# TravisWheelerLab/BATH

Hardware: AMD Instinct MI355X
Metric: DP Gcells/s + residues/s through bathsearch pipeline at 1/2/4/8 MI355X (higher is better)
Workload: dtype u8/i16 integer scores (SSV: exact binary16), f32 Forward

## Files before the change

### bath_amd/csrc/bath_common.hpp

```cpp
#pragma once
#include <set>
#include <atomic>
#include <hip/hip_runtime.h>

#include <cstdint>
#include <chrono>
#include <cstdio>
#include <cstdlib>
#include <cstring>
#include <condition_variable>
#include <functional>
#include <mutex>
#include <shared_mutex>
#include <string>
#include <thread>
#include <vector>

#include "bath_hip.h"

namespace bath {

inline hipError_t allow_max_lds(const void *fn) {
  static std::mutex mu;
  static std::set<std::pair<int, const void *>> done;
  int dev = 0;
  (void)hipGetDevice(&dev);
  std::lock_guard<std::mutex> g(mu);
  if (done.count({dev, fn})) return hipSuccess;
  hipFuncAttributes at{};
  size_t fixed = 0;
  if (hipFuncGetAttributes(&at, fn) == hipSuccess) fixed = at.sharedSizeBytes; else (void)hipGetLastError();
  const hipError_t e = hipFuncSetAttribute(fn, hipFuncAttributeMaxDynamicSharedMemorySize, (int)(160 * 1024 - (int)std::min<size_t>(fixed, 96 * 1024)));
  if (e == hipSuccess) done.insert({dev, fn});
  return e;
}

constexpr int kKp = BATH_KP_AMINO;
constexpr int kRowReset = 29;
constexpr int kSsvRows = 30;
constexpr int kStop = 27;
constexpr int kXaa = 26;
constexpr int kOrfBins = 2048;
constexpr int kOrfCursorStride = 32;
constexpr int kOrfMiscInts = (1 + kOrfCursorStride) * kOrfBins + 64;

#define BATH_HIP_TRY(ctx, call)                                                            \
  do {                                                                                     \
    hipError_t e_ = (call);                                                                \
    if (e_ != hipSuccess) {                                                                \
      (ctx)->set_error(std::string(#call) + ": " + hipGetErrorString(e_));                 \
      return BATH_EFAIL;                                                                   \
    }                                                                                      \
  } while (0)

struct DevBuf {
  void *p = nullptr;
  size_t cap = 0;
  hipError_t reserve(size_t bytes) {
    if (bytes <= cap) return hipSuccess;
    if (p) (void)hipFree(p);
    p = nullptr; cap = 0;
    size_t want = bytes + bytes / 4 + 256;
// ... 246 lines not shown
  uint64_t uid = 0;
  int M = 0, max_length = 0, L0 = 0;
  float nj = 1.f;
  float evparam[BATH_NEVPARAM];
  float compo[BATH_K_AMINO];
  std::vector<uint8_t> rb;
  std::vector<int16_t> rw;
  std::vector<int16_t> tw;
  std::vector<float> rf, tf;
  uint8_t tbm_b = 0, tec_b = 0, base_b = 0, bias_b = 0;
  float scale_b = 0;
  int16_t xw_E[2] = {0, 0};
  float scale_w = 0;
  int16_t base_w = 0, ddbound_w = 0;
  float xf_E[2] = {0, 0};
  std::string consensus;
  std::vector<uint8_t> cons_digital;
  uint8_t *d_cons = nullptr;
  std::vector<float> prefix_lengths, suffix_lengths;
  int NR = 0, G = 1;
  int ssv_row_bytes = 0;
  int16_t *d_ssv = nullptr;
  int16_t *d_msv = nullptr;
  uint8_t *d_rb = nullptr;
  int rb_stride = 0;
  int16_t *d_rw = nullptr;
  int16_t *d_tw = nullptr;
  float *d_rf = nullptr, *d_tf = nullptr;
  float *d_rfb = nullptr, *d_tfb = nullptr;
  float *d_msc = nullptr, *d_tsc = nullptr;
  float *d_bias_eo = nullptr;
  int vit_NR = 0, vit_rw_pitch = 0;
  int16_t *d_vit_rw = nullptr; uint32_t *d_vit_tw2 = nullptr; int16_t *d_vit_rank = nullptr;
  mutable LenTables lt;
  mutable std::mutex grow_mu;
  mutable std::vector<void *> retired;
  mutable int16_t *d_emit = nullptr;
  mutable double emit_F1 = -1.0;
  mutable int emit_maxlen = -1;
  int ensure_len_tables(int maxL) const;
};

namespace bath {
int build_len_tables(const bath_hip_oprofile *om, int maxL);
void bias_filter_eo(const float *compo, float eo[kKp][2]);
double gumbel_surv(double x, double mu, double lambda);
// ... 15 lines not shown
```

### bath_amd/csrc/bath_filters.hip

```cpp
#include <cmath>
#include <cstring>
#include <algorithm>
#include <numeric>

#include "bath_common.hpp"
#include "bath_kernels.hpp"
#include "bath_launch.hpp"

using namespace bath;

namespace bath {


template <int NR, int G>
__global__ __launch_bounds__(256, NR <= 76 ? 4 : 1) void ssv_lane_kernel(SeqView sq, const int32_t *__restrict__ order,
                                                       const int16_t *__restrict__ cost_tab, int row_bytes,
                                                       int16_t *__restrict__ out_v) {
  extern __shared__ __attribute__((aligned(16))) char lds[];
  {
    const int n32 = kSsvRows * row_bytes / 4;
    const uint32_t *src = reinterpret_cast<const uint32_t *>(cost_tab);
    uint32_t *dst = reinterpret_cast<uint32_t *>(lds);
    for (int i = threadIdx.x; i < n32; i += blockDim.x) dst[i] = src[i];
  }
  __syncthreads();
  const int64_t gt = (int64_t)blockIdx.x * blockDim.x + threadIdx.x;
  const int lane_ = threadIdx.x & 63;
  const int64_t t = (gt >> 6) * (64 / G) + SsvGroups<G>::slot(lane_);
  const int grank = SsvGroups<G>::rank(lane_);
  const bool live = t < sq.n;
  const int64_t sid = live ? (order ? (int64_t)order[t] : t) : 0;
  const int L = live ? sq.len[sid] : 0;
  const uint8_t *s = sq.data + sq.off[sid];
  const int Lw = wave_max_i32(L);
  const char *tile = lds + grank * (4 * NR);
  const unsigned tile_addr = (unsigned)(size_t)(__attribute__((address_space(3))) const char *)tile;

  s16x2 reg[NR];
  const s16x2 fl = {0, 0};
#pragma unroll
  for (int r = 0; r < NR; r++) reg[r] = fl;
  s16x2 xE = fl, xE2 = fl;

  uint32_t wnext = (0 < L) ? *reinterpret_cast<const uint32_t *>(s) : 0x1d1d1d1du;
  for (int i0 = 0; i0 < Lw; i0 += 4) {
    const uint32_t w = wnext;
    wnext = (i0 + 4 < L) ? *reinterpret_cast<const uint32_t *>(s + i0 + 4) : 0x1d1d1d1du;
#pragma unroll 1
    for (int j = 0; j < 4; j++) {
      int x = (w >> (8 * j)) & 0xff;
      x = (i0 + j < L) ? min(x, kKp - 1) : kRowReset;
      const unsigned carry = ssv_carry<NR, G>(reg, grank);
      ssv_row_pipe<NR, 3>(reg, xE, xE2, tile_addr + (unsigned)(x * row_bytes), carry);
    }
  }
  xE = ssv_max3(xE, xE2, xE2);
  const int v = ssv_group_max<G>(xE);
  if (live && grank == 0) out_v[sid] = (int16_t)min(v, 32767);
}

__global__ void ssv_classify_kernel(int64_t n, const int32_t *__restrict__ len, const int16_t *__restrict__ v,
                                    const uint8_t *__restrict__ tjb_tab, MsvConsts c, float *__restrict__ sc,
                                    int32_t *__restrict__ status) {
  const int64_t t = (int64_t)blockIdx.x * blockDim.x + threadIdx.x;
  if (t >= n) return;
  float s = 0.f;
  const int st = ssv_classify(v[t], tjb_tab[len[t]], c, &s);
  sc[t] = s;
  status[t] = st;
}

template <int C>
__global__ __launch_bounds__(256) void msv_wave_kernel(SeqView sq, int M, const uint8_t *__restrict__ rb, int rb_stride,
                                                       const uint8_t *__restrict__ tjb_tab, MsvConsts c,
                                                       const int32_t *__restrict__ todo, int64_t ntodo, const int *__restrict__ ntodo_dev,
                                                       float *__restrict__ sc, int32_t *__restrict__ status) {
// ... 576 lines not shown
  c.base_w = om->base_w; c.xwE_loop = om->xw_E[0]; c.xwE_move = om->xw_E[1]; c.scale_w = om->scale_w;
  c.scale_b = om->scale_b; c.base_b = om->base_b; c.tec_b = om->tec_b; c.bias_b = om->bias_b;
  c.Q8 = std::max(2, ((om->M - 1) / 8) + 1);
  return c;
}

static int length_order(bath_hip_ctx *ctx, const bath_hip_seqs *sq, DevBuf &buf) {
  std::vector<int32_t> order((size_t)sq->n);
  std::iota(order.begin(), order.end(), 0);
  std::stable_sort(order.begin(), order.end(), [&](int32_t a, int32_t b) { return sq->h_len[a] > sq->h_len[b]; });
  BATH_HIP_TRY(ctx, buf.reserve(order.size() * sizeof(int32_t) + 16));
  BATH_HIP_TRY(ctx, hipMemcpyAsync(buf.p, order.data(), order.size() * sizeof(int32_t), hipMemcpyHostToDevice, ctx->stream));
  return BATH_OK;
}

int launch_ssv_lane(bath_hip_ctx *ctx, const bath_hip_oprofile *om, SeqView v, const int32_t *d_order, int16_t *d_v) {
  if (v.n == 0) return BATH_OK;
  const int G = om->G;
  const size_t shmem = (size_t)kSsvRows * om->ssv_row_bytes;
  const int threads = 256;
  const int blocks = (int)((v.n * G + threads - 1) / threads);
  const int rb = om->ssv_row_bytes;
  bool launched = false;
#define BATH_SSV_CASE(N, GG)                                                                                             \
  if (!launched && om->NR == N && G == GG) {                                                                             \
    if (shmem > 64 * 1024) (void)bath::allow_max_lds((const void *)ssv_lane_kernel<N, GG>); \
    hipLaunchKernelGGL((ssv_lane_kernel<N, GG>), dim3(blocks), dim3(threads), shmem, ctx->stream, v, d_order, om->d_ssv, rb, d_v); \
    launched = true;                                                                                                     \
  }
  BATH_SSV_SHAPES(BATH_SSV_CASE)
#undef BATH_SSV_CASE
  if (!launched) { ctx->set_error("SSV kernel: no tile shape for model length " + std::to_string(om->M)); return BATH_EINVAL; }
  BATH_HIP_TRY(ctx, hipGetLastError());
  return BATH_OK;
}

constexpr size_t kWaveTableLdsMax = 150 * 1024;

static int columns_per_lane(int M) {
  int c = (M + 63) / 64;
  for (int opt : {1, 2, 3, 4, 6, 8, 12, 16, 24, 32}) if (c <= opt) return opt;
  return -1;
}

#define BATH_C_SWITCH(C, BODY)                                   \
  switch (C) {                                                   \
    case 1: { constexpr int CC = 1; BODY } break;                \
    case 2: { constexpr int CC = 2; BODY } break;                \
    case 3: { constexpr int CC = 3; BODY } break;                \
    case 4: { constexpr int CC = 4; BODY } break;                \
// ... 225 lines not shown
```

### bath_amd/csrc/bath_kernels.hpp

```cpp
#pragma once
#include <climits>
#include <hip/hip_runtime.h>

#include <cstdint>

#include "bath_hip.h"

namespace bath {

typedef short s16x2 __attribute__((ext_vector_type(2)));

template <int CTRL, int ROW_MASK = 0xf>
__device__ __forceinline__ int dpp_i(int v, int old) { return __builtin_amdgcn_update_dpp(old, v, CTRL, ROW_MASK, 0xf, false); }
__device__ __forceinline__ int wave_shr1_i32(int v, int fill) { return dpp_i<0x138>(v, fill); }
__device__ __forceinline__ float wave_shr1_f32(float v, float fill) {
  return __builtin_bit_cast(float, __builtin_amdgcn_update_dpp(__builtin_bit_cast(int, fill), __builtin_bit_cast(int, v), 0x138, 0xf, 0xf, false));
}
__device__ __forceinline__ float wave_max_f32(float v) {
  const int ninf = (int)0xff800000;
#define BATH_FMAX_STEP(CTRL, MASK) v = fmaxf(v, __builtin_bit_cast(float, __builtin_amdgcn_update_dpp(ninf, __builtin_bit_cast(int, v), CTRL, MASK, 0xf, false)));
  BATH_FMAX_STEP(0x111, 0xf) BATH_FMAX_STEP(0x112, 0xf) BATH_FMAX_STEP(0x114, 0xf) BATH_FMAX_STEP(0x118, 0xf) BATH_FMAX_STEP(0x142, 0xa) BATH_FMAX_STEP(0x143, 0xc)
#undef BATH_FMAX_STEP
  return __builtin_bit_cast(float, __builtin_amdgcn_readlane(__builtin_bit_cast(int, v), 63));
}
// ... 17 lines not shown
  BATH_FSUM_STEP(0x111, 0xf) BATH_FSUM_STEP(0x112, 0xf) BATH_FSUM_STEP(0x114, 0xf) BATH_FSUM_STEP(0x118, 0xf) BATH_FSUM_STEP(0x142, 0xa) BATH_FSUM_STEP(0x143, 0xc)
#undef BATH_FSUM_STEP
  return __builtin_bit_cast(float, __builtin_amdgcn_readlane(__builtin_bit_cast(int, v), 63));
#endif
}
__device__ __forceinline__ int sat16(int v) { return min(max(v, -32768), 32767); }
__device__ __forceinline__ int satu8(int v) { return min(max(v, 0), 255); }


constexpr unsigned kSsvBeginPair = 0x00000000u;

__device__ __forceinline__ s16x2 ssv_add(s16x2 a, int inc) {
  s16x2 r;
  asm("v_pk_add_f16 %0, %1, %2 clamp" : "=v"(r) : "v"(a), "v"(inc));
  return r;
}
__device__ __forceinline__ s16x2 ssv_max3(s16x2 a, s16x2 b, s16x2 c) {
  s16x2 r;
  asm("v_pk_maximum3_f16 %0, %1, %2, %3" : "=v"(r) : "v"(a), "v"(b), "v"(c));
  return r;
}

typedef int ssv_i4 __attribute__((ext_vector_type(4)));
template <int N> __device__ __forceinline__ void ssv_lgkm_wait(ssv_i4 &c) {
  if (N <= 0) asm volatile("s_waitcnt lgkmcnt(0)" : "+v"(c));
  else if (N == 1) asm volatile("s_waitcnt lgkmcnt(1)" : "+v"(c));
  else asm volatile("s_waitcnt lgkmcnt(2)" : "+v"(c));
}
template <int NR, int NB, int g, int US = 16>
struct SsvRowPipe {
  static constexpr int NG = NR / 4;
  static __device__ __forceinline__ void run(s16x2 (&reg)[NR], s16x2 &xE, s16x2 &xE2, unsigned rowaddr, s16x2 wrap, ssv_i4 (&b)[NB]) {
    constexpr int r = NR - 4 - 4 * g;
    ssv_i4 &c = b[g % NB];
    ssv_lgkm_wait<(NG - 1 - g < NB - 1) ? NG - 1 - g : NB - 1>(c);
    const s16x2 v3 = ssv_add(reg[r + 2], c.w);
    const s16x2 v2 = ssv_add(reg[r + 1], c.z);
    reg[r + 3] = v3;
    reg[r + 2] = v2;
    xE = ssv_max3(xE, v3, v2);
    const s16x2 v1 = ssv_add(reg[r], c.y);
    const s16x2 v0 = ssv_add((r > 0) ? reg[r - 1] : wrap, c.x);
    reg[r + 1] = v1;
    reg[r] = v0;
    xE2 = ssv_max3(xE2, v1, v0);
    if (g + NB < NG) {
      asm volatile("ds_read_b128 %0, %1 offset:%2" : "=v"(c) : "v"(rowaddr), "n"(US * ((NR - 4 - 4 * (g + NB)) / 4)), "v"(v0), "v"(v1));
    }
    SsvRowPipe<NR, NB, g + 1, US>::run(reg, xE, xE2, rowaddr, wrap, b);
  }
};
template <int NR, int NB, int US>
struct SsvRowPipe<NR, NB, NR / 4, US> {
  static __device__ __forceinline__ void run(s16x2 (&)[NR], s16x2 &, s16x2 &, unsigned, s16x2, ssv_i4 (&)[NB]) {}
};
template <int NR, int NB = 2, int US = 16>
__device__ __forceinline__ void ssv_row_pipe(s16x2 (&reg)[NR], s16x2 &xE, s16x2 &xE2, unsigned rowaddr , unsigned carry) {
  static_assert(NR % 4 == 0 && NR >= 4 * NB && NB >= 2 && NB <= 3, "registers are consumed four at a time (one 16-byte LDS read)");
  const s16x2 wrap = __builtin_bit_cast(s16x2, __builtin_amdgcn_alignbit(__builtin_bit_cast(unsigned, reg[NR - 1]), carry, 16));
  ssv_i4 b[NB];
  asm volatile("ds_read_b128 %0, %1 offset:%2" : "=v"(b[0]) : "v"(rowaddr), "n"(US * ((NR - 4) / 4)));
  asm volatile("ds_read_b128 %0, %1 offset:%2" : "=v"(b[1]) : "v"(rowaddr), "n"(US * ((NR - 8) / 4)));
  if (NB > 2) asm volatile("ds_read_b128 %0, %1 offset:%2" : "=v"(b[NB - 1]) : "v"(rowaddr), "n"(US * ((NR - 12) / 4)));
  SsvRowPipe<NR, NB, 0, US>::run(reg, xE, xE2, rowaddr, wrap, b);
}

template <int G> struct SsvGroups {
  static constexpr int TPW = 64 / G;
  static __device__ __forceinline__ int rank(int lane) { return lane / TPW; }
  static __device__ __forceinline__ int slot(int lane) { return lane % TPW; }
};
template <int NR, int G>
__device__ __forceinline__ unsigned ssv_carry(const s16x2 (&reg)[NR], int grank) {
  if (G == 1) return kSsvBeginPair;
  const unsigned far = (unsigned)__shfl_up((int)__builtin_bit_cast(unsigned, reg[NR - 1]), SsvGroups<G>::TPW, 64);
  return (grank == 0) ? kSsvBeginPair : far;
}
template <int G>
__device__ __forceinline__ int ssv_group_max(s16x2 xE) {
  typedef _Float16 h16x2 __attribute__((ext_vector_type(2)));
  const h16x2 h = __builtin_bit_cast(h16x2, xE);
  int v = (int)(fmaxf((float)h.x, (float)h.y) * 2048.0f) - 128;
#pragma unroll
  for (int d = SsvGroups<G>::TPW; d < 64; d <<= 1) v = max(v, __shfl_xor(v, d, 64));
  return v;
}

struct MsvConsts {
  int tbm, tec, base, bias;
  float scale_b;
};

__device__ __forceinline__ int ssv_classify(int v, int tjb, const MsvConsts &c, float *sc) {
  if (tjb + c.tbm + c.tec + c.bias >= 127) return BATH_ENORESULT;
  unsigned xE = (v >= -1 - c.bias) ? 255u : (unsigned)(v + 256);
  if ((int)xE >= 255 - c.bias) {
    *sc = INFINITY;
    return (c.base - tjb - c.tbm < 128) ? BATH_ENORESULT : BATH_ERANGE;
// ... 47 lines not shown
```

### bath_amd/csrc/bath_launch.hpp

```cpp
#pragma once
#include <functional>
#include <utility>

#include "bath_common.hpp"

#define BATH_SSV_SHAPES(X)                                                                                   \
  X(16, 1) X(20, 1) X(24, 1) X(28, 1) X(32, 1) X(36, 1) X(40, 1) X(44, 1) X(48, 1) X(52, 1) X(56, 1) X(60, 1) X(64, 1)     \
  X(68, 1) X(72, 1) X(76, 1) X(80, 1) X(84, 1) X(88, 1) X(92, 1) X(96, 1) X(100, 1) X(104, 1) X(108, 1) X(112, 1)           \
  X(128, 1) X(144, 1) X(160, 1) X(176, 1) X(192, 1) X(208, 1)                                                \
  X(40, 2) X(48, 2) X(56, 2) X(64, 2) X(72, 2) X(76, 2)                                                     \
  X(112, 2) X(128, 2) X(144, 2) X(160, 2) X(176, 2) X(192, 2) X(208, 2)                                      \
  X(112, 4) X(128, 4) X(144, 4) X(160, 4) X(176, 4) X(192, 4) X(208, 4)                                      \
  X(112, 8) X(128, 8) X(144, 8) X(160, 8) X(176, 8) X(192, 8) X(208, 8)

namespace bath {

struct Cand {
  int64_t *window;  int32_t *sf;
  int32_t *startj;  int32_t *len;
  int16_t *v;
  int64_t *off;
  int32_t *msv_status, *vit_status, *fwd_status, *stage, *flags;
  float *usc, *nullsc, *filtersc, *vfsc, *fwdsc;
  double *P;
  int32_t *kminmax;
};

int build_orf_records(bath_hip_ctx *ctx, const Cand &cand, int nc, int64_t window_offset, bath_orf_result **d_out, int64_t *n_out);

struct VitWindowArgs {
  double invP_vit, invP_msv;
  const float *d_filtersc;
  const uint8_t *d_ssv_scores;
  void *d_wins;
  int *d_win_count;
  int win_cap;
// ... 124 lines not shown
```

### bath_amd/csrc/bath_msv_lane.hip

```cpp
#include "bath_common.hpp"
#include "bath_kernels.hpp"
#include "bath_launch.hpp"

using namespace bath;

namespace bath {

__device__ __forceinline__ s16x2 msv_pkmax(s16x2 a, s16x2 b) {
  s16x2 r;
  asm("v_pk_max_f16 %0, %1, %2" : "=v"(r) : "v"(a), "v"(b));
  return r;
}

template <int NR>
__global__ __launch_bounds__(256, NR <= 76 ? 4 : 1) void msv_lane_kernel(SeqView sq, const int16_t *__restrict__ cost_tab , int row_bytes,
                                                                        const uint8_t *__restrict__ tjb_tab, MsvConsts c,
                                                                        const int32_t *__restrict__ todo, int64_t ntodo, const int *__restrict__ ntodo_dev,
                                                                        float *__restrict__ sc, int32_t *__restrict__ status) {
  extern __shared__ __attribute__((aligned(16))) char lds[];
  {
    const int n32 = kSsvRows * row_bytes / 4;
    const uint32_t *src = reinterpret_cast<const uint32_t *>(cost_tab);
    uint32_t *dst = reinterpret_cast<uint32_t *>(lds);
    for (int i = threadIdx.x; i < n32; i += blockDim.x) dst[i] = src[i];
// ... 50 lines not shown
        xE2 = ssv_max3(xE2, v1, v0);
      }
      const h16x2 e1 = __builtin_bit_cast(h16x2, xE), e2 = __builtin_bit_cast(h16x2, xE2);
      int xEi = (int)(fmaxf(fmaxf((float)e1.x, (float)e1.y), fmaxf((float)e2.x, (float)e2.y)) * 2048.0f);
      if (xEi + c.bias >= 255) overflow = true;
      xEi = max(xEi - c.tec, 0);
      xJ = max(xJ, xEi);
      xB = max(max(c.base, xJ) - tjbm, 0);
    }
    if (live) {
      if (overflow) { sc[sid] = INFINITY; status[sid] = BATH_ERANGE; }
      else {
        float r = ((float)(xJ - tjb) - (float)c.base);
        r /= c.scale_b;
        r = (float)((double)r - 3.0);
        sc[sid] = r; status[sid] = BATH_OK;
      }
    }
  }
}

int launch_msv_lane(bath_hip_ctx *ctx, const bath_hip_oprofile *om, SeqView v, const int32_t *d_todo, int64_t ntodo, float *d_sc, int32_t *d_status, const int *ntodo_dev) {
  static const bool off = [] { const char *e = std::getenv("BATH_HIP_MSV_WAVE"); return e && e[0] == '1'; }();
  if (off || om->G != 1 || om->NR > 76 || !om->d_msv) return BATH_ENORESULT;
  if (ntodo == 0) return BATH_OK;
  const size_t shmem = (size_t)kSsvRows * om->ssv_row_bytes;
  const int64_t waves = (ntodo + 63) / 64;
  const int grid = (int)std::max<int64_t>(1, std::min<int64_t>((waves + 3) / 4, (int64_t)ctx->prop.multiProcessorCount * 4));
  bool launched = false;
#define BATH_MSV_CASE(N)                                                                                                               \
  if (!launched && om->NR == N) {                                                                                                      \
    hipLaunchKernelGGL((msv_lane_kernel<N>), dim3(grid), dim3(256), shmem, ctx->stream, v, om->d_msv, om->ssv_row_bytes, om->lt.d_tjb,   \
                       MsvConsts{om->tbm_b, om->tec_b, om->base_b, om->bias_b, om->scale_b}, d_todo, ntodo, ntodo_dev, d_sc, d_status); \
    launched = true;                                                                                                                   \
  }
  BATH_MSV_CASE(16) BATH_MSV_CASE(20) BATH_MSV_CASE(24) BATH_MSV_CASE(28) BATH_MSV_CASE(32) BATH_MSV_CASE(36) BATH_MSV_CASE(40) BATH_MSV_CASE(44)
  BATH_MSV_CASE(48) BATH_MSV_CASE(52) BATH_MSV_CASE(56) BATH_MSV_CASE(60) BATH_MSV_CASE(64) BATH_MSV_CASE(68) BATH_MSV_CASE(72) BATH_MSV_CASE(76)
#undef BATH_MSV_CASE
  if (!launched) return BATH_ENORESULT;
  BATH_HIP_TRY(ctx, hipGetLastError());
  return BATH_OK;
}

}
```

### bath_amd/csrc/bath_pipeline.hip

```cpp
#include <algorithm>
#include <cmath>
#include <cstring>
#include <cstdlib>
#include <map>
#include <thread>

#include "bath_common.hpp"
#include "bath_kernels.hpp"
#include "bath_launch.hpp"
#include "host_model.hpp"

using namespace bath;

namespace bath {

static const double kLog2 = 0.69314718055994529;
constexpr int kVitLongOrf = 128;

enum { FLAG_VIT_RUN = 1, FLAG_HAS_WIN = 2 };

struct Counters {
  int cand_count, todo_msv, todo_vit, todo_ssvb, todo_vit2, todo_fwd, win_count, overflow;
  int todo_lb, pad_;
  unsigned long long n_orfs, orf_res;
  unsigned long long n_past_msv, n_past_bias, n_past_vit, n_past_fwd;
  unsigned long long pos_past_msv, pos_past_bias, pos_past_vit, pos_past_fwd;
  unsigned long long res_vit, res_fwd;
  unsigned long long res_seen;
};

struct Params {
  double F1, F2, F3, F4;
  int do_bias, fs_pipe, minlen;
  float evparam[BATH_NEVPARAM];
};

template <int NR, int G>
__global__ __launch_bounds__(256, NR <= 76 ? 4 : 1) void ssv_orf_kernel(const uint8_t *__restrict__ aa, const OrfRec *__restrict__ orfs, const int *__restrict__ n_orfs_dev,
                                                      SeqView dna, const int16_t *__restrict__ cost_tab, int row_bytes,
                                                      const int16_t *__restrict__ emit_thresh, int thresh_max,
                                                      Cand cand, int cand_cap, Counters *__restrict__ ctr, int chunk) {
  extern __shared__ __attribute__((aligned(16))) char lds[];
  if (chunk > 0 && (int64_t)blockIdx.x * (blockDim.x >> 6) * chunk * (64 / G) >= (int64_t)*n_orfs_dev) return;
  {
    const int n32 = kSsvRows * row_bytes / 4;
    const uint32_t *src = reinterpret_cast<const uint32_t *>(cost_tab);
    uint32_t *dst = reinterpret_cast<uint32_t *>(lds);
    for (int i = threadIdx.x; i < n32; i += blockDim.x) dst[i] = src[i];
  }
  __syncthreads();
  constexpr int TPW = 64 / G;
  const int64_t n_orfs = *n_orfs_dev;
  const int lane = threadIdx.x & 63;
  const int grank = SsvGroups<G>::rank(lane);
  const char *tile = lds + grank * (4 * NR);
  const unsigned tile_addr = (unsigned)(size_t)(__attribute__((address_space(3))) const char *)tile;
  const int64_t wave0 = ((int64_t)blockIdx.x * blockDim.x + threadIdx.x) >> 6;
  const int64_t nwaves = ((int64_t)gridDim.x * blockDim.x) >> 6;
  const s16x2 fl = {0, 0};
  const int64_t tb_first = chunk > 0 ? wave0 * chunk * TPW : wave0 * TPW, tb_step = chunk > 0 ? TPW : nwaves * TPW;
  const int64_t tb_end = chunk > 0 ? (tb_first + (int64_t)chunk * TPW < n_orfs ? tb_first + (int64_t)chunk * TPW : n_orfs) : n_orfs;
  for (int64_t tb = tb_first; tb < tb_end; tb += tb_step) {
    const int64_t t = tb + SsvGroups<G>::slot(lane);
    const bool live = t < n_orfs;
    OrfRec rec{0, 0, 0};
    if (live) rec = orfs[t];
    const int L = rec.len_sf & 0x0fffffff;
#ifdef BATH_SSV_POOL_PROBE
    const uint8_t *s = aa + ((size_t)(tb / TPW) * 8192) % ((size_t)1 << 27) + (size_t)lane * 8;
#define BATH_SSV_RES(i8) (s + (size_t)(i8) * 64)
#else
    const uint8_t *s = aa + rec.aa_off;
#define BATH_SSV_RES(i8) (s + (i8))
#endif
    const int Lw = wave_max_i32(L);
    s16x2 reg[NR];
#pragma unroll
    for (int r = 0; r < NR; r++) reg[r] = fl;
    s16x2 xE = fl, xE2 = fl;
    uint64_t qnext = (0 < L) ? *reinterpret_cast<const uint64_t *>(BATH_SSV_RES(0)) : 0x1d1d1d1d1d1d1d1dull;
    for (int i0 = 0; i0 < Lw; i0 += 8) {
      const uint64_t q = qnext;
      qnext = (i0 + 8 < L) ? *reinterpret_cast<const uint64_t *>(BATH_SSV_RES(i0 + 8)) : 0x1d1d1d1d1d1d1d1dull;
      const int nrow = min(8, Lw - i0);
      for (int h = 0; h < 2; h++) {
        const uint32_t qh = h ? (uint32_t)(q >> 32) : (uint32_t)q;
        const int nh = min(4, nrow - 4 * h);
        for (int j = 0; j < nh; j++) {
          int x = (int)__builtin_amdgcn_ubfe(qh, 8 * j, 8);
          x = (i0 + 4 * h + j < L) ? x : kRowReset;
          const unsigned carry = ssv_carry<NR, G>(reg, grank);
          ssv_row_pipe<NR, 3>(reg, xE, xE2, tile_addr + __umul24((unsigned)x, (unsigned)row_bytes), carry);
        }
      }
    }
    xE = ssv_max3(xE, xE2, xE2);
    const int v = ssv_group_max<G>(xE);
    if (dna.context) {
      unsigned long long r = 0;
      if (live && grank == 0) {
        const int sf = (int)((unsigned)rec.len_sf >> 28);
        const int64_t w = rec.w;
        const int startj = (int32_t)(rec.aa_off - (2 * dna.off[w] + 96 * w + (int64_t)sf * orf_stream_pitch(dna.len[w])));
        const int C = dna.context[w], start_s = sf % 3 + 3 * startj + 1;
        if (sf < 3 ? (start_s + 3 * L - 1 < C) : (dna.len[w] - start_s + 1 < C)) r = (unsigned long long)L;
      }
      if (__ballot(r != 0)) { for (int d = 32; d >= 1; d >>= 1) r += __shfl_xor(r, d, 64); if (lane == 0) atomicAdd(&ctr->res_seen, r); }
    }
    if (live && grank == 0 && v >= (int)emit_thresh[min(L, thresh_max)]) {
      const int sf = (int)((unsigned)rec.len_sf >> 28);
      const int64_t w = rec.w;
      const int64_t stream = 2 * dna.off[w] + 96 * w + (int64_t)sf * orf_stream_pitch(dna.len[w]);
      const int startj = (int32_t)(rec.aa_off - stream);
      bool seen = false;
      if (dna.context) {
        const int C = dna.context[w], start_s = sf % 3 + 3 * startj + 1;
        seen = sf < 3 ? (start_s + 3 * L - 1 < C) : (dna.len[w] - start_s + 1 < C);
      }
      const int slot = seen ? cand_cap + 1 : atomicAdd(&ctr->cand_count, 1);
      if (seen) {
// ... 517 lines not shown
  if (ssv_shmem > 160 * 1024) { ctx->set_error("model too long for the LDS-resident SSV cost table"); return BATH_EINVAL; }
  const int dec_blocks = ctx->prop.multiProcessorCount * 4;

  std::vector<hipEvent_t> &ev = ctx->ev_pool;
  while (ev.size() < 12) { hipEvent_t e; BATH_HIP_TRY(ctx, hipEventCreate(&e)); ev.push_back(e); }

  PipelineWork W;
  Counters hc{};
  int win_need = 0;
  for (int attempt = 0;; attempt++) {
    size_t need = layout(W, nullptr, (int)cap, win_need);
    BATH_HIP_TRY(ctx, b_work.reserve(need + 4096));
    layout(W, b_work.as<char>(), (int)cap, win_need);
    W.pool = b_aa.as<uint8_t>();
    BATH_HIP_TRY(ctx, hipMemsetAsync(W.ctr, 0, sizeof(Counters), ctx->stream));
    SeqView cv{W.pool, W.cand.off, W.cand.len, cap};

    int e = 0;
    BATH_HIP_TRY(ctx, hipEventRecord(ev[e++], ctx->stream));
    if ((st = launch_orf_scan(ctx, dna, tt, prm->min_orf_len, ob, &W.ctr->n_orfs, &W.ctr->orf_res, prm->strands)) != BATH_OK) return st;
    BATH_HIP_TRY(ctx, hipEventRecord(ev[e++], ctx->stream));
    {
      static const int ssv_chunk = [] { const char *e = std::getenv("BATH_HIP_SSV_CHUNK"); return e ? std::atoi(e) : 0; }();
      int blocks = ctx->prop.multiProcessorCount * 4;
      const int ssv_threads = 256;
      const int wpb = ssv_threads / 64;
      if (ssv_chunk > 0) blocks = (int)std::min<int64_t>((max_orfs + (int64_t)wpb * (64 / om->G) * ssv_chunk - 1) / ((int64_t)wpb * (64 / om->G) * ssv_chunk), 1 << 30);
      bool launched = false;
#define BATH_ORF_CASE(N, GG)                                                                                                     \
  if (!launched && NRk == N && om->G == GG) {                                                                                    \
    if (ssv_shmem > 64 * 1024) (void)bath::allow_max_lds((const void *)ssv_orf_kernel<N, GG>); \
    hipLaunchKernelGGL((ssv_orf_kernel<N, GG>), dim3(blocks), dim3(ssv_threads), ssv_shmem, ctx->stream, W.pool, ob.sorted, ob.ntotal,                  \
                       dna->view(), om->d_ssv, om->ssv_row_bytes, d_emit, max_orf, W.cand, W.cand_cap, W.ctr, ssv_chunk);        \
    launched = true;                                                                                                             \
  }
      BATH_SSV_SHAPES(BATH_ORF_CASE)
#undef BATH_ORF_CASE
      if (!launched) { ctx->set_error("SSV kernel: no tile shape for this model length"); return BATH_EINVAL; }
      BATH_HIP_TRY(ctx, hipGetLastError());
    }
    BATH_HIP_TRY(ctx, hipEventRecord(ev[e++], ctx->stream));
    hipStream_t bulk_stream = ctx->stream;
    struct StreamRestore { bath_hip_ctx *c; hipStream_t s; ~StreamRestore() { c->stream = s; } } stream_restore{ctx, bulk_stream};
    if (ctx->tail_stream) {
      BATH_HIP_TRY(ctx, hipStreamWaitEvent(ctx->tail_stream, ev[e - 1], 0));
      ctx->stream = ctx->tail_stream;
    }
    static const int64_t lane_min_nt = [] { const char *e = std::getenv("BATH_HIP_LANE_MIN_NT"); return e ? std::atoll(e) : (int64_t)150'000'000; }();
    const bool few_cands = dna->total < lane_min_nt, few_msv = dna->total < 2 * lane_min_nt;
    hipLaunchKernelGGL(classify_kernel, dim3(dec_blocks), dim3(256), 0, ctx->stream, W.cand, W.cand_cap, W.ctr, om->lt.d_tjb, mc, W.todo_msv);
    BATH_HIP_TRY(ctx, hipGetLastError());
    if ((st = launch_msv_wave(ctx, om, cv, W.todo_msv, cap, W.cand.usc, W.cand.msv_status, &W.ctr->todo_msv, !few_msv)) != BATH_OK) return st;
    BATH_HIP_TRY(ctx, hipEventRecord(ev[e++], ctx->stream));
    hipLaunchKernelGGL(f1_bias_kernel, dim3(dec_blocks), dim3(256), 0, ctx->stream, W.cand, W.cand_cap, W.ctr, P, W.pool, M, om->d_bias_eo,
                       om->lt.d_nullsc, om->lt.d_p1, om->lt.d_lt1, om->lt.d_lt2, W.todo_vit, W.todo_ssvb);
// ... 949 lines not shown
```

### bath_amd/csrc/bath_profile.hip

```cpp
#include <atomic>
#include <cctype>
#include <cmath>
#include <cstring>

#include "bath_common.hpp"
#include "host_model.hpp"

using namespace bath;

namespace bath {

static const double kLog2 = 0.69314718055994529;

double gumbel_surv(double x, double mu, double lambda) {
  double ey = -std::exp(-lambda * (x - mu));
  if (std::fabs(ey) < 5e-9) return -ey;
  return 1.0 - std::exp(ey);
}
double gumbel_invsurv(double p, double mu, double lambda) {
  double lp = (p < 5e-9) ? (std::pow(p, p) - 1) / p : std::log(-1. * std::log(1 - p));
  return mu - lp / lambda;
}
double exp_surv(double x, double mu, double lambda) { return (x < mu) ? 1.0 : std::exp(-lambda * (x - mu)); }

// ... 280 lines not shown
    for (int s : {MD, MI, II, DD}) t[s] = (k < M) ? expf(tsc(k, s)) : 0.f;
  }
  om->xf_E[0] = expf(gm->xsc[0][0]);
  om->xf_E[1] = expf(gm->xsc[0][1]);

  {
    std::vector<float> &pre = om->prefix_lengths, &suf = om->suffix_lengths;
    pre.assign(W, 0.f); suf.assign(W, 0.f);
    float total = 0;
    for (int k = 1; k < M; k++) {
      const float t_mi = om->tf[(size_t)k * 8 + MI], t_ii = om->tf[(size_t)k * 8 + II];
      pre[k] = (t_mi == 0) ? 1.f : (float)(1 + (int)(std::log(1e-7 / t_mi) / std::log((double)t_ii)));
      total += pre[k];
    }
    pre[0] = pre[M] = 0;
    for (int k = 1; k < M; k++) pre[k] /= total;
    suf[M] = pre[M - 1];
    for (int k = M - 1; k >= 1; k--) suf[k] = suf[k + 1] + pre[k - 1];
    for (int k = 2; k < M; k++) pre[k] += pre[k - 1];
  }

  static const bool wide = [] { const char *e = std::getenv("BATH_HIP_SSV_WIDE"); return e && e[0] == '1'; }();
  static const int g2max = [] { const char *e = std::getenv("BATH_HIP_SSV_G2_MAX"); return e ? std::atoi(e) : 304; }();
  int G = (!wide && M > 152 && M <= g2max) ? 2 : 1;
  while (G < 8 && M > 416 * G) G *= 2;
  if (M > 416 * G) { ctx->set_error("model longer than 3328 nodes"); delete om; return BATH_EINVAL; }
  int NR = ((M + G - 1) / G + 1) / 2;
  if (G == 1 && NR <= 112) NR = (NR + 3) / 4 * 4;
  else if (G == 2 && NR <= 76) NR = NR <= 40 ? 40 : (NR <= 72 ? (NR + 7) / 8 * 8 : 76);
  else NR = std::max((NR + 15) / 16 * 16, G > 1 ? 112 : 16);
  NR = std::max(NR, 16);
  om->NR = NR; om->G = G;
  om->ssv_row_bytes = 16 * ((NR * G / 4 + 1) | 1);
  {
    size_t rowsz = (size_t)om->ssv_row_bytes / 2;
    auto half_bits = [](float v) { const _Float16 h = (_Float16)v; int16_t b; std::memcpy(&b, &h, 2); return b; };
    std::vector<int16_t> tab((size_t)kSsvRows * rowsz, half_bits(-1.0f));
    for (int x = 0; x < kKp; x++)
      for (int k = 1; k <= M; k++) {
        const int g = (k - 1) / (2 * NR), q = (k - 1) - g * 2 * NR;
        const int cost = std::min((int)om->rb[x * W + k] - (int)om->bias_b, 127);
        tab[x * rowsz + (size_t)g * 2 * NR + 2 * (q % NR) + q / NR] = half_bits(-(float)cost / 2048.0f);
      }
    BATH_HIP_TRY(ctx, upload(&om->d_ssv, tab.data(), tab.size(), ctx->stream));
    if (G == 1 && NR <= 76) {
      std::vector<int16_t> mtab((size_t)kSsvRows * rowsz, half_bits(-1.0f));
      for (int x = 0; x < kKp; x++)
        for (int k = 1; k <= M; k++) {
          const int q = k - 1;
          const int inc = (int)om->bias_b - (int)om->rb[x * W + k];
          mtab[x * rowsz + 2 * (q % NR) + q / NR] = half_bits((float)inc / 2048.0f);
        }
      BATH_HIP_TRY(ctx, upload(&om->d_msv, mtab.data(), mtab.size(), ctx->stream));
    }
  }
  {
    int NRv = ((M + 1) / 2 + 15) / 16 * 16;
    if (NRv == 80) NRv = std::max(68, ((M + 1) / 2 + 3) / 4 * 4);
    if (NRv <= 112) {
      om->vit_NR = NRv;
      om->vit_rw_pitch = 4 * NRv + 16;
      const size_t rowsz = (size_t)om->vit_rw_pitch / 2;
      std::vector<int16_t> rwt((size_t)30 * rowsz, (int16_t)-32768);
      auto slot = [&](int node) { return node <= NRv ? 2 * (node - 1) : 2 * (node - NRv - 1) + 1; };
      for (int x = 0; x < kKp; x++)
        for (int k = 1; k <= M; k++) rwt[x * rowsz + slot(k)] = om->rw[x * W + k];
      std::vector<uint32_t> tw2((size_t)NRv * 8);
      std::vector<int16_t> rank((size_t)2 * NRv, (int16_t)32767);
      const int Q8 = std::max(2, ((M - 1) / 8) + 1);
      auto twv = [&](int node, int s) -> int { return node <= M ? (int)om->tw[(size_t)node * 8 + s] : -32768; };
      for (int r = 0; r < NRv; r++)
        for (int s = 0; s < 8; s++) tw2[(size_t)r * 8 + s] = ((uint32_t)(uint16_t)twv(r + 1, s)) | ((uint32_t)(uint16_t)twv(NRv + r + 1, s) << 16);
      for (int node = 1; node <= M; node++) rank[(size_t)slot(node)] = (int16_t)(((node - 1) % Q8) * 8 + (node - 1) / Q8);
      BATH_HIP_TRY(ctx, upload(&om->d_vit_rw, rwt.data(), rwt.size(), ctx->stream));
// ... 249 lines not shown
```

Before: 197.2 billion.

## Allow non-multiple-of-4 SSV register counts and add G=2 high-occupancy shapes

```diff
diff --git a/bath_amd/csrc/bath_common.hpp b/bath_amd/csrc/bath_common.hpp
--- a/bath_amd/csrc/bath_common.hpp
+++ b/bath_amd/csrc/bath_common.hpp
@@ -38,6 +38,7 @@
 constexpr int kKp = BATH_KP_AMINO;
 constexpr int kRowReset = 29;
 constexpr int kSsvRows = 30;
+__host__ __device__ constexpr int ssv_tile_regs(int NR) { return (NR + 3) / 4 * 4; }
 constexpr int kStop = 27;
 constexpr int kXaa = 26;
 constexpr int kOrfBins = 2048;
@@ -330,6 +331,7 @@
   int ssv_row_bytes = 0;
   int16_t *d_ssv = nullptr;
   int16_t *d_msv = nullptr;
+  int msv_NR = 0, msv_row_bytes = 0;
   uint8_t *d_rb = nullptr;
   int rb_stride = 0;
   int16_t *d_rw = nullptr;
diff --git a/bath_amd/csrc/bath_filters.hip b/bath_amd/csrc/bath_filters.hip
--- a/bath_amd/csrc/bath_filters.hip
+++ b/bath_amd/csrc/bath_filters.hip
@@ -12,8 +12,8 @@
 namespace bath {
 
 
-template <int NR, int G>
-__global__ __launch_bounds__(256, NR <= 76 ? 4 : 1) void ssv_lane_kernel(SeqView sq, const int32_t *__restrict__ order,
+template <int NR, int G, int W>
+__global__ __launch_bounds__(256, W) void ssv_lane_kernel(SeqView sq, const int32_t *__restrict__ order,
                                                        const int16_t *__restrict__ cost_tab, int row_bytes,
                                                        int16_t *__restrict__ out_v) {
   extern __shared__ __attribute__((aligned(16))) char lds[];
@@ -33,7 +33,7 @@
   const int L = live ? sq.len[sid] : 0;
   const uint8_t *s = sq.data + sq.off[sid];
   const int Lw = wave_max_i32(L);
-  const char *tile = lds + grank * (4 * NR);
+  const char *tile = lds + grank * (4 * ssv_tile_regs(NR));
   const unsigned tile_addr = (unsigned)(size_t)(__attribute__((address_space(3))) const char *)tile;
 
   s16x2 reg[NR];
@@ -51,7 +51,7 @@
       int x = (w >> (8 * j)) & 0xff;
       x = (i0 + j < L) ? min(x, kKp - 1) : kRowReset;
       const unsigned carry = ssv_carry<NR, G>(reg, grank);
-      ssv_row_pipe<NR, 3>(reg, xE, xE2, tile_addr + (unsigned)(x * row_bytes), carry);
+      ssv_row_pipe<NR, (W >= 6 ? 2 : 3)>(reg, xE, xE2, tile_addr + (unsigned)(x * row_bytes), carry);
     }
   }
   xE = ssv_max3(xE, xE2, xE2);
@@ -674,10 +674,10 @@
   const int blocks = (int)((v.n * G + threads - 1) / threads);
   const int rb = om->ssv_row_bytes;
   bool launched = false;
-#define BATH_SSV_CASE(N, GG)                                                                                             \
+#define BATH_SSV_CASE(N, GG, WW)                                                                                         \
   if (!launched && om->NR == N && G == GG) {                                                                             \
-    if (shmem > 64 * 1024) (void)bath::allow_max_lds((const void *)ssv_lane_kernel<N, GG>); \
-    hipLaunchKernelGGL((ssv_lane_kernel<N, GG>), dim3(blocks), dim3(threads), shmem, ctx->stream, v, d_order, om->d_ssv, rb, d_v); \
+    if (shmem > 64 * 1024) (void)bath::allow_max_lds((const void *)ssv_lane_kernel<N, GG, WW>); \
+    hipLaunchKernelGGL((ssv_lane_kernel<N, GG, WW>), dim3(blocks), dim3(threads), shmem, ctx->stream, v, d_order, om->d_ssv, rb, d_v); \
     launched = true;                                                                                                     \
   }
   BATH_SSV_SHAPES(BATH_SSV_CASE)
diff --git a/bath_amd/csrc/bath_kernels.hpp b/bath_amd/csrc/bath_kernels.hpp
--- a/bath_amd/csrc/bath_kernels.hpp
+++ b/bath_amd/csrc/bath_kernels.hpp
@@ -63,15 +63,21 @@
 }
 
 typedef int ssv_i4 __attribute__((ext_vector_type(4)));
-template <int N> __device__ __forceinline__ void ssv_lgkm_wait(ssv_i4 &c) {
+typedef int ssv_i2 __attribute__((ext_vector_type(2)));
+template <int N, typename T> __device__ __forceinline__ void ssv_lgkm_wait(T &c) {
   if (N <= 0) asm volatile("s_waitcnt lgkmcnt(0)" : "+v"(c));
   else if (N == 1) asm volatile("s_waitcnt lgkmcnt(1)" : "+v"(c));
   else asm volatile("s_waitcnt lgkmcnt(2)" : "+v"(c));
 }
+template <int NR> struct SsvTail { typedef ssv_i2 T; };
+template <> struct SsvTail<0> { typedef int T; };
 template <int NR, int NB, int g, int US = 16>
 struct SsvRowPipe {
-  static constexpr int NG = NR / 4;
-  static __device__ __forceinline__ void run(s16x2 (&reg)[NR], s16x2 &xE, s16x2 &xE2, unsigned rowaddr, s16x2 wrap, ssv_i4 (&b)[NB]) {
+  static constexpr int NF = NR / 4;
+  static constexpr int NG = (NR + 3) / 4;
+  static constexpr int PAD = ssv_tile_regs(NR) - NR;
+  typedef typename SsvTail<NR % 4 == 1 ? 0 : 1>::T Tail;
+  static __device__ __forceinline__ void run(s16x2 (&reg)[NR], s16x2 &xE, s16x2 &xE2, unsigned rowaddr, s16x2 wrap, ssv_i4 (&b)[NB], Tail &tl) {
     constexpr int r = NR - 4 - 4 * g;
     ssv_i4 &c = b[g % NB];
     ssv_lgkm_wait<(NG - 1 - g < NB - 1) ? NG - 1 - g : NB - 1>(c);
@@ -85,25 +91,46 @@
     reg[r + 1] = v1;
     reg[r] = v0;
     xE2 = ssv_max3(xE2, v1, v0);
-    if (g + NB < NG) {
-      asm volatile("ds_read_b128 %0, %1 offset:%2" : "=v"(c) : "v"(rowaddr), "n"(US * ((NR - 4 - 4 * (g + NB)) / 4)), "v"(v0), "v"(v1));
-    }
-    SsvRowPipe<NR, NB, g + 1, US>::run(reg, xE, xE2, rowaddr, wrap, b);
+    if (g + NB < NF)
+      asm volatile("ds_read_b128 %0, %1 offset:%2" : "=v"(c) : "v"(rowaddr), "n"(US * ((NR - 4 - 4 * (g + NB) + PAD) / 4)), "v"(v0), "v"(v1));
+    else if (g + NB < NG && NR % 4 == 1)
+      asm volatile("ds_read_b32 %0, %1 offset:%2" : "=v"(tl) : "v"(rowaddr), "n"(4 * PAD), "v"(v0), "v"(v1));
+    else if (g + NB < NG)
+      asm volatile("ds_read_b64 %0, %1 offset:%2" : "=v"(tl) : "v"(rowaddr), "n"(4 * PAD), "v"(v0), "v"(v1));
+    SsvRowPipe<NR, NB, g + 1, US>::run(reg, xE, xE2, rowaddr, wrap, b, tl);
   }
 };
 template <int NR, int NB, int US>
 struct SsvRowPipe<NR, NB, NR / 4, US> {
-  static __device__ __forceinline__ void run(s16x2 (&)[NR], s16x2 &, s16x2 &, unsigned, s16x2, ssv_i4 (&)[NB]) {}
+  typedef typename SsvTail<NR % 4 == 1 ? 0 : 1>::T Tail;
+  static __device__ __forceinline__ void run(s16x2 (&reg)[NR], s16x2 &, s16x2 &xE2, unsigned, s16x2 wrap, ssv_i4 (&)[NB], Tail &tl) {
+    if constexpr (NR % 4 == 1) {
+      ssv_lgkm_wait<0>(tl);
+      const s16x2 v0 = ssv_add(wrap, tl);
+      reg[0] = v0;
+      xE2 = ssv_max3(xE2, v0, v0);
+    } else if constexpr (NR % 4 == 2) {
+      ssv_lgkm_wait<0>(tl);
+      const s16x2 v1 = ssv_add(reg[0], tl.y);
+      const s16x2 v0 = ssv_add(wrap, tl.x);
+      reg[1] = v1;
+      reg[0] = v0;
+      xE2 = ssv_max3(xE2, v1, v0);
+    }
+  }
 };
 template <int NR, int NB = 2, int US = 16>
 __device__ __forceinline__ void ssv_row_pipe(s16x2 (&reg)[NR], s16x2 &xE, s16x2 &xE2, unsigned rowaddr , unsigned carry) {
-  static_assert(NR % 4 == 0 && NR >= 4 * NB && NB >= 2 && NB <= 3, "registers are consumed four at a time (one 16-byte LDS read)");
+  static_assert((NR % 4 == 0 || ((NR % 4 == 1 || NR % 4 == 2) && US == 16)) && NR / 4 >= NB && NB >= 2 && NB <= 3,
+                "registers are consumed four at a time (one 16-byte LDS read), the last one or two of NR = 4n + 1 / 4n + 2 with one 4- / 8-byte read");
+  constexpr int PAD = ssv_tile_regs(NR) - NR;
   const s16x2 wrap = __builtin_bit_cast(s16x2, __builtin_amdgcn_alignbit(__builtin_bit_cast(unsigned, reg[NR - 1]), carry, 16));
   ssv_i4 b[NB];
-  asm volatile("ds_read_b128 %0, %1 offset:%2" : "=v"(b[0]) : "v"(rowaddr), "n"(US * ((NR - 4) / 4)));
-  asm volatile("ds_read_b128 %0, %1 offset:%2" : "=v"(b[1]) : "v"(rowaddr), "n"(US * ((NR - 8) / 4)));
-  if (NB > 2) asm volatile("ds_read_b128 %0, %1 offset:%2" : "=v"(b[NB - 1]) : "v"(rowaddr), "n"(US * ((NR - 12) / 4)));
-  SsvRowPipe<NR, NB, 0, US>::run(reg, xE, xE2, rowaddr, wrap, b);
+  typename SsvRowPipe<NR, NB, 0, US>::Tail tl;
+  asm volatile("ds_read_b128 %0, %1 offset:%2" : "=v"(b[0]) : "v"(rowaddr), "n"(US * ((NR - 4 + PAD) / 4)));
+  asm volatile("ds_read_b128 %0, %1 offset:%2" : "=v"(b[1]) : "v"(rowaddr), "n"(US * ((NR - 8 + PAD) / 4)));
+  if (NB > 2) asm volatile("ds_read_b128 %0, %1 offset:%2" : "=v"(b[NB - 1]) : "v"(rowaddr), "n"(US * ((NR - 12 + PAD) / 4)));
+  SsvRowPipe<NR, NB, 0, US>::run(reg, xE, xE2, rowaddr, wrap, b, tl);
 }
 
 template <int G> struct SsvGroups {
@@ -114,7 +141,13 @@
 template <int NR, int G>
 __device__ __forceinline__ unsigned ssv_carry(const s16x2 (&reg)[NR], int grank) {
   if (G == 1) return kSsvBeginPair;
-  const unsigned far = (unsigned)__shfl_up((int)__builtin_bit_cast(unsigned, reg[NR - 1]), SsvGroups<G>::TPW, 64);
+  const unsigned last = __builtin_bit_cast(unsigned, reg[NR - 1]);
+  unsigned far;
+  if (G == 2) {
+    far = (unsigned)__builtin_amdgcn_permlane32_swap(last, last, false, false)[0];
+  } else {
+    far = (unsigned)__shfl_up((int)last, SsvGroups<G>::TPW, 64);
+  }
   return (grank == 0) ? kSsvBeginPair : far;
 }
 template <int G>
diff --git a/bath_amd/csrc/bath_launch.hpp b/bath_amd/csrc/bath_launch.hpp
--- a/bath_amd/csrc/bath_launch.hpp
+++ b/bath_amd/csrc/bath_launch.hpp
@@ -4,14 +4,19 @@
 
 #include "bath_common.hpp"
 
-#define BATH_SSV_SHAPES(X)                                                                                   \
-  X(16, 1) X(20, 1) X(24, 1) X(28, 1) X(32, 1) X(36, 1) X(40, 1) X(44, 1) X(48, 1) X(52, 1) X(56, 1) X(60, 1) X(64, 1)     \
-  X(68, 1) X(72, 1) X(76, 1) X(80, 1) X(84, 1) X(88, 1) X(92, 1) X(96, 1) X(100, 1) X(104, 1) X(108, 1) X(112, 1)           \
-  X(128, 1) X(144, 1) X(160, 1) X(176, 1) X(192, 1) X(208, 1)                                                \
-  X(40, 2) X(48, 2) X(56, 2) X(64, 2) X(72, 2) X(76, 2)                                                     \
-  X(112, 2) X(128, 2) X(144, 2) X(160, 2) X(176, 2) X(192, 2) X(208, 2)                                      \
-  X(112, 4) X(128, 4) X(144, 4) X(160, 4) X(176, 4) X(192, 4) X(208, 4)                                      \
-  X(112, 8) X(128, 8) X(144, 8) X(160, 8) X(176, 8) X(192, 8) X(208, 8)
+#define BATH_SSV_SHAPES(X)                                                                                                 \
+  X(16, 1, 4) X(17, 1, 4) X(18, 1, 4) X(20, 1, 4) X(21, 1, 4) X(22, 1, 4) X(24, 1, 4) X(25, 1, 4) X(26, 1, 4) X(28, 1, 4)  \
+  X(29, 1, 4) X(30, 1, 4) X(32, 1, 4) X(33, 1, 4) X(34, 1, 4) X(36, 1, 4) X(37, 1, 4) X(38, 1, 4) X(40, 1, 4) X(41, 1, 4)  \
+  X(42, 1, 4) X(44, 1, 4) X(45, 1, 4) X(46, 1, 4) X(48, 1, 4) X(49, 1, 4) X(50, 1, 4) X(52, 1, 4) X(53, 1, 4) X(54, 1, 4)  \
+  X(56, 1, 4) X(57, 1, 4) X(58, 1, 4) X(60, 1, 4) X(61, 1, 4) X(62, 1, 4) X(64, 1, 4) X(65, 1, 4) X(66, 1, 4) X(68, 1, 4)  \
+  X(69, 1, 4) X(70, 1, 4) X(72, 1, 4) X(73, 1, 4) X(74, 1, 4) X(76, 1, 4)                                                  \
+  X(80, 1, 1) X(84, 1, 1) X(88, 1, 1) X(92, 1, 1) X(96, 1, 1) X(100, 1, 1) X(104, 1, 1) X(108, 1, 1) X(112, 1, 1)           \
+  X(128, 1, 1) X(144, 1, 1) X(160, 1, 1) X(176, 1, 1) X(192, 1, 1) X(208, 1, 1)                                             \
+  X(32, 2, 6) X(34, 2, 6) X(36, 2, 6) X(38, 2, 6)                                                               \
+  X(40, 2, 4) X(48, 2, 4) X(56, 2, 4) X(64, 2, 4) X(72, 2, 4) X(76, 2, 4)                                                   \
+  X(112, 2, 1) X(128, 2, 1) X(144, 2, 1) X(160, 2, 1) X(176, 2, 1) X(192, 2, 1) X(208, 2, 1)                                \
+  X(112, 4, 1) X(128, 4, 1) X(144, 4, 1) X(160, 4, 1) X(176, 4, 1) X(192, 4, 1) X(208, 4, 1)                                \
+  X(112, 8, 1) X(128, 8, 1) X(144, 8, 1) X(160, 8, 1) X(176, 8, 1) X(192, 8, 1) X(208, 8, 1)
 
 namespace bath {
 
diff --git a/bath_amd/csrc/bath_msv_lane.hip b/bath_amd/csrc/bath_msv_lane.hip
--- a/bath_amd/csrc/bath_msv_lane.hip
+++ b/bath_amd/csrc/bath_msv_lane.hip
@@ -96,15 +96,15 @@
 
 int launch_msv_lane(bath_hip_ctx *ctx, const bath_hip_oprofile *om, SeqView v, const int32_t *d_todo, int64_t ntodo, float *d_sc, int32_t *d_status, const int *ntodo_dev) {
   static const bool off = [] { const char *e = std::getenv("BATH_HIP_MSV_WAVE"); return e && e[0] == '1'; }();
-  if (off || om->G != 1 || om->NR > 76 || !om->d_msv) return BATH_ENORESULT;
+  if (off || !om->d_msv) return BATH_ENORESULT;
   if (ntodo == 0) return BATH_OK;
-  const size_t shmem = (size_t)kSsvRows * om->ssv_row_bytes;
+  const size_t shmem = (size_t)kSsvRows * om->msv_row_bytes;
   const int64_t waves = (ntodo + 63) / 64;
   const int grid = (int)std::max<int64_t>(1, std::min<int64_t>((waves + 3) / 4, (int64_t)ctx->prop.multiProcessorCount * 4));
   bool launched = false;
 #define BATH_MSV_CASE(N)                                                                                                               \
-  if (!launched && om->NR == N) {                                                                                                      \
-    hipLaunchKernelGGL((msv_lane_kernel<N>), dim3(grid), dim3(256), shmem, ctx->stream, v, om->d_msv, om->ssv_row_bytes, om->lt.d_tjb,   \
+  if (!launched && om->msv_NR == N) {                                                                                                      \
+    hipLaunchKernelGGL((msv_lane_kernel<N>), dim3(grid), dim3(256), shmem, ctx->stream, v, om->d_msv, om->msv_row_bytes, om->lt.d_tjb,   \
                        MsvConsts{om->tbm_b, om->tec_b, om->base_b, om->bias_b, om->scale_b}, d_todo, ntodo, ntodo_dev, d_sc, d_status); \
     launched = true;                                                                                                                   \
   }
diff --git a/bath_amd/csrc/bath_pipeline.hip b/bath_amd/csrc/bath_pipeline.hip
--- a/bath_amd/csrc/bath_pipeline.hip
+++ b/bath_amd/csrc/bath_pipeline.hip
@@ -35,8 +35,8 @@
   float evparam[BATH_NEVPARAM];
 };
 
-template <int NR, int G>
-__global__ __launch_bounds__(256, NR <= 76 ? 4 : 1) void ssv_orf_kernel(const uint8_t *__restrict__ aa, const OrfRec *__restrict__ orfs, const int *__restrict__ n_orfs_dev,
+template <int NR, int G, int W>
+__global__ __launch_bounds__(256, W) void ssv_orf_kernel(const uint8_t *__restrict__ aa, const OrfRec *__restrict__ orfs, const int *__restrict__ n_orfs_dev,
                                                       SeqView dna, const int16_t *__restrict__ cost_tab, int row_bytes,
                                                       const int16_t *__restrict__ emit_thresh, int thresh_max,
                                                       Cand cand, int cand_cap, Counters *__restrict__ ctr, int chunk) {
@@ -53,7 +53,7 @@
   const int64_t n_orfs = *n_orfs_dev;
   const int lane = threadIdx.x & 63;
   const int grank = SsvGroups<G>::rank(lane);
-  const char *tile = lds + grank * (4 * NR);
+  const char *tile = lds + grank * (4 * ssv_tile_regs(NR));
   const unsigned tile_addr = (unsigned)(size_t)(__attribute__((address_space(3))) const char *)tile;
   const int64_t wave0 = ((int64_t)blockIdx.x * blockDim.x + threadIdx.x) >> 6;
   const int64_t nwaves = ((int64_t)gridDim.x * blockDim.x) >> 6;
@@ -61,16 +61,17 @@
   const int64_t tb_first = chunk > 0 ? wave0 * chunk * TPW : wave0 * TPW, tb_step = chunk > 0 ? TPW : nwaves * TPW;
   const int64_t tb_end = chunk > 0 ? (tb_first + (int64_t)chunk * TPW < n_orfs ? tb_first + (int64_t)chunk * TPW : n_orfs) : n_orfs;
   for (int64_t tb = tb_first; tb < tb_end; tb += tb_step) {
-    const int64_t t = tb + SsvGroups<G>::slot(lane);
-    const bool live = t < n_orfs;
-    OrfRec rec{0, 0, 0};
-    if (live) rec = orfs[t];
-    const int L = rec.len_sf & 0x0fffffff;
+    int L = 0;
+    int64_t aa_off = 0;
+    {
+      const int64_t t = tb + SsvGroups<G>::slot(lane);
+      if (t < n_orfs) { L = orfs[t].len_sf & 0x0fffffff; aa_off = orfs[t].aa_off; }
+    }
 #ifdef BATH_SSV_POOL_PROBE
     const uint8_t *s = aa + ((size_t)(tb / TPW) * 8192) % ((size_t)1 << 27) + (size_t)lane * 8;
 #define BATH_SSV_RES(i8) (s + (size_t)(i8) * 64)
 #else
-    const uint8_t *s = aa + rec.aa_off;
+    const uint8_t *s = aa + aa_off;
 #define BATH_SSV_RES(i8) (s + (i8))
 #endif
     const int Lw = wave_max_i32(L);
@@ -90,12 +91,18 @@
           int x = (int)__builtin_amdgcn_ubfe(qh, 8 * j, 8);
           x = (i0 + 4 * h + j < L) ? x : kRowReset;
           const unsigned carry = ssv_carry<NR, G>(reg, grank);
-          ssv_row_pipe<NR, 3>(reg, xE, xE2, tile_addr + __umul24((unsigned)x, (unsigned)row_bytes), carry);
+          ssv_row_pipe<NR, (W >= 6 ? 2 : 3)>(reg, xE, xE2, tile_addr + __umul24((unsigned)x, (unsigned)row_bytes), carry);
         }
       }
     }
     xE = ssv_max3(xE, xE2, xE2);
     const int v = ssv_group_max<G>(xE);
+    const int64_t t = tb + SsvGroups<G>::slot(lane);
+    const bool live = t < n_orfs;
+    const OrfRec *orfs_again = orfs;
+    asm volatile("" : "+s"(orfs_again));
+    OrfRec rec{0, 0, 0};
+    if (live) rec = orfs_again[t];
     if (dna.context) {
       unsigned long long r = 0;
       if (live && grank == 0) {
@@ -659,15 +666,15 @@
     BATH_HIP_TRY(ctx, hipEventRecord(ev[e++], ctx->stream));
     {
       static const int ssv_chunk = [] { const char *e = std::getenv("BATH_HIP_SSV_CHUNK"); return e ? std::atoi(e) : 0; }();
-      int blocks = ctx->prop.multiProcessorCount * 4;
+      int blocks = 0;
       const int ssv_threads = 256;
       const int wpb = ssv_threads / 64;
       if (ssv_chunk > 0) blocks = (int)std::min<int64_t>((max_orfs + (int64_t)wpb * (64 / om->G) * ssv_chunk - 1) / ((int64_t)wpb * (64 / om->G) * ssv_chunk), 1 << 30);
       bool launched = false;
-#define BATH_ORF_CASE(N, GG)                                                                                                     \
+#define BATH_ORF_CASE(N, GG, WW)                                                                                                 \
   if (!launched && NRk == N && om->G == GG) {                                                                                    \
-    if (ssv_shmem > 64 * 1024) (void)bath::allow_max_lds((const void *)ssv_orf_kernel<N, GG>); \
-    hipLaunchKernelGGL((ssv_orf_kernel<N, GG>), dim3(blocks), dim3(ssv_threads), ssv_shmem, ctx->stream, W.pool, ob.sorted, ob.ntotal,                  \
+    if (ssv_shmem > 64 * 1024) (void)bath::allow_max_lds((const void *)ssv_orf_kernel<N, GG, WW>); \
+    hipLaunchKernelGGL((ssv_orf_kernel<N, GG, WW>), dim3(blocks > 0 ? blocks : ctx->prop.multiProcessorCount * WW), dim3(ssv_threads), ssv_shmem, ctx->stream, W.pool, ob.sorted, ob.ntotal,                  \
                        dna->view(), om->d_ssv, om->ssv_row_bytes, d_emit, max_orf, W.cand, W.cand_cap, W.ctr, ssv_chunk);        \
     launched = true;                                                                                                             \
   }
diff --git a/bath_amd/csrc/bath_profile.hip b/bath_amd/csrc/bath_profile.hip
--- a/bath_amd/csrc/bath_profile.hip
+++ b/bath_amd/csrc/bath_profile.hip
@@ -326,16 +326,21 @@
 
   static const bool wide = [] { const char *e = std::getenv("BATH_HIP_SSV_WIDE"); return e && e[0] == '1'; }();
   static const int g2max = [] { const char *e = std::getenv("BATH_HIP_SSV_G2_MAX"); return e ? std::atoi(e) : 304; }();
-  int G = (!wide && M > 152 && M <= g2max) ? 2 : 1;
+  static const int narrow_min = [] { const char *e = std::getenv("BATH_HIP_SSV_NARROW_MIN"); return e ? std::atoi(e) : 153; }();
+  int G = (!wide && M >= narrow_min && M <= g2max) ? 2 : 1;
   while (G < 8 && M > 416 * G) G *= 2;
   if (M > 416 * G) { ctx->set_error("model longer than 3328 nodes"); delete om; return BATH_EINVAL; }
   int NR = ((M + G - 1) / G + 1) / 2;
-  if (G == 1 && NR <= 112) NR = (NR + 3) / 4 * 4;
+  if (G == 1 && NR <= 76) NR += (NR % 4 == 3);
+  else if (G == 1 && NR <= 112) NR = (NR + 3) / 4 * 4;
+  else if (G == 2 && NR <= 38) NR = std::max(32, (NR + 1) / 2 * 2);
   else if (G == 2 && NR <= 76) NR = NR <= 40 ? 40 : (NR <= 72 ? (NR + 7) / 8 * 8 : 76);
   else NR = std::max((NR + 15) / 16 * 16, G > 1 ? 112 : 16);
   NR = std::max(NR, 16);
   om->NR = NR; om->G = G;
-  om->ssv_row_bytes = 16 * ((NR * G / 4 + 1) | 1);
+  const int NRt = ssv_tile_regs(NR);
+  om->ssv_row_bytes = 16 * ((NRt * G / 4 + 1) | 1);
+  const int msv_NR = std::max(16, ((M + 1) / 2 + 3) / 4 * 4);
   {
     size_t rowsz = (size_t)om->ssv_row_bytes / 2;
     auto half_bits = [](float v) { const _Float16 h = (_Float16)v; int16_t b; std::memcpy(&b, &h, 2); return b; };
@@ -344,16 +349,19 @@
       for (int k = 1; k <= M; k++) {
         const int g = (k - 1) / (2 * NR), q = (k - 1) - g * 2 * NR;
         const int cost = std::min((int)om->rb[x * W + k] - (int)om->bias_b, 127);
-        tab[x * rowsz + (size_t)g * 2 * NR + 2 * (q % NR) + q / NR] = half_bits(-(float)cost / 2048.0f);
+        tab[x * rowsz + (size_t)g * 2 * NRt + 2 * (NRt - NR + q % NR) + q / NR] = half_bits(-(float)cost / 2048.0f);
       }
     BATH_HIP_TRY(ctx, upload(&om->d_ssv, tab.data(), tab.size(), ctx->stream));
-    if (G == 1 && NR <= 76) {
-      std::vector<int16_t> mtab((size_t)kSsvRows * rowsz, half_bits(-1.0f));
+    if (msv_NR <= 76) {
+      om->msv_NR = msv_NR;
+      om->msv_row_bytes = 16 * ((msv_NR / 4 + 1) | 1);
+      const size_t mrowsz = (size_t)om->msv_row_bytes / 2;
+      std::vector<int16_t> mtab((size_t)kSsvRows * mrowsz, half_bits(-1.0f));
       for (int x = 0; x < kKp; x++)
         for (int k = 1; k <= M; k++) {
           const int q = k - 1;
           const int inc = (int)om->bias_b - (int)om->rb[x * W + k];
-          mtab[x * rowsz + 2 * (q % NR) + q / NR] = half_bits((float)inc / 2048.0f);
+          mtab[x * mrowsz + 2 * (q % msv_NR) + q / msv_NR] = half_bits((float)inc / 2048.0f);
         }
       BATH_HIP_TRY(ctx, upload(&om->d_msv, mtab.data(), mtab.size(), ctx->stream));
     }
```

Result: faster. 199.2 billion, median of 6 (+1.0%).
